# tky823/audio_source_separation

Hardware: AMD Instinct MI355X
Metric: ILRMA iterations/sec (4ch, F=1025, T=4096) (higher is better)
Workload: dtype f64; 1 GPU; gauss_ilrma_ip update_once, M=4 F=1025 T=4096 K=4, normalize=power, loss off; utterances_per_gpu=1, power_statistic=covariance, parallelism=utterance-sharded x1, no data-path collective

## Files before the change

### audio_source_separation_amd/csrc/assx_bss.hip

```cpp
#include "assx_common.hpp"
#include "assx_small_linalg.hpp"
#include "assx_stream.hpp"
#include "assx_group_linalg.hpp"
#include "assx_partition.hpp"
#include "assx_cov_wide.hpp"
#include "assx_cov_mfma.hpp"
#include "assx_nmf_internal.hpp"
#include "assx_widem.hpp"

using namespace assx;

namespace {

constexpr int REDUCE_THREADS = 256;

template <typename R, int M>
__device__ __forceinline__ void load_filter(const Cx<R>* __restrict__ W, size_t bf, Cx<R> (&w)[M][M]) {
  const Cx<R>* p = W + bf * (M * M);
#pragma unroll
  for (int n = 0; n < M; ++n)
#pragma unroll
    for (int m = 0; m < M; ++m) w[n][m] = p[n * M + m];
}

// ... 701 lines not shown
    for (int n = 0; n < N; ++n)
      Xi[((size_t)b * N + n) * FT + (size_t)(f0 + j) * T + t] =
          fma(nu, floor_eps<R>(r[n][j], eps), (R)2 * cabs2(y[n])) * inv;
  }
}

template <typename R>
__global__ void __launch_bounds__(256) pow_map_kernel(const R* __restrict__ in, R* __restrict__ out, size_t n, PowSpec p) {
  const size_t i = (size_t)blockIdx.x * blockDim.x + threadIdx.x;
  if (i < n) out[i] = powspec<R>(in[i], p);
}
template <typename R>
__global__ void __launch_bounds__(256) mix_variance_kernel(const R* __restrict__ Lambda, const R* __restrict__ g,
                                                          R* __restrict__ out, int M, int N, int F, int T) {
  const int t = blockIdx.x * blockDim.x + threadIdx.x, f = blockIdx.y, b = blockIdx.z;
  if (t >= T) return;
  const size_t FT = (size_t)F * T;
  for (int m = 0; m < M; ++m) {
    R acc = 0;
    for (int n = 0; n < N; ++n)
      acc += Lambda[((size_t)b * N + n) * FT + (size_t)f * T + t] * g[(((size_t)b * N + n) * F + f) * M + m];
    out[((size_t)b * M + m) * FT + (size_t)f * T + t] = acc;
  }
}

struct WsLayout {
  size_t part;
  size_t u;
  size_t lpart;
  size_t small;
  size_t map;
  size_t nmf;
  size_t tmp;
  size_t total;
};

constexpr int CHIP_CUS = 256;

inline long long g_target(int wgs_per_cu) {
  static const int rounds = lab_int("ASSX_ROUNDS", 1);
  const int forced = knob_int("ASSX_G", 0);
  if (forced > 0) return forced;
  return (long long)CHIP_CUS * wgs_per_cu * (rounds < 1 ? 1 : rounds);
}

inline int tblocks(int T) { return (T + WAVE - 1) / WAVE; }

template <typename R, int M>
constexpr int cov_lane_split() { return 1; }
inline FlatPart flat_cov(int B, int F, int T, int LS) {
  const int fb = WAVE / LS, tbk = (T + fb - 1) / fb;
  return make_flat(B, (long long)F * tbk, tbk, g_target(8));
}
inline FlatPart flat_basis(int B, int F, int T) {
  return make_flat(B, (long long)F * tblocks(T), tblocks(T), g_target(8));
}
inline FlatPart flat_act(int B, int F, int T) {
  return make_flat(B, (long long)tblocks(T) * F, F, g_target(8 / ACT_NH));
}

inline FlatPart flat_cov_wide(int B, int F, int T, int sb = 1) {
  const int tbk = (T + WAVE * sb - 1) / (WAVE * sb);
  return make_flat(B, (long long)((F + COVW_BINS - 1) / COVW_BINS) * tbk, tbk, g_target(1));
}
template <typename R>
inline int cov_wide_sb(int NK) {
// ... 22 lines not shown
  size_t pmax = p_cov;
  if (K > KU) {
    for (int sb = 1; sb <= 2; ++sb) {
      const FlatPart fw = flat_cov_wide(B, F, T, sb);
      const size_t p_wide = (size_t)fw.G * fw.S * COVW_BINS * (M * M * M);
      if (p_wide > pmax) pmax = p_wide;
    }
    const size_t p_adapt = (size_t)B * tblocks(T) * M * 2 * Kc * WAVE;
    if (p_adapt > pmax) pmax = p_adapt;
  }
  if (p_basis > pmax) pmax = p_basis;
  if (p_act > pmax) pmax = p_act;
  if (p_pb > pmax) pmax = p_pb;
  if (p_pow > pmax) pmax = p_pow;
  if (p_aux > pmax) pmax = p_aux;
  WsLayout L;
  L.part = 0;
  size_t off = align_up(pmax * r, 256);
  L.u = off;
  off += align_up((size_t)B * M * F * M * M * 2 * r, 256);
  L.lpart = off;
  size_t nl = (size_t)B * ((size_t)TS * F + (size_t)M * F + (size_t)M * ((T + 63) / 64) + F + 16 +
                           (size_t)flat_loss(F, T).G);
  off += align_up(nl * 8, 256);
  L.small = off;
  off += align_up((size_t)B * (M + 8) * 8, 256);
  L.map = L.nmf = L.tmp = off;
  if (K > KU) {
    off += align_up((size_t)B * M * F * T * r, 256);
    L.nmf = off;
    off += align_up(assx_nmf_workspace_bytes(B * M, F, T, K, dtype), 256);
    L.tmp = off;
    off += align_up(((size_t)B * M * F * K + (size_t)B * M * K * T) * r, 256);
  }
  L.total = off;
  return L;
}

template <typename Fn>
int dispatch_rm(assx_ctx* ctx, int dtype, int M, Fn&& fn) {
  if (dtype == ASSX_F64) {
    switch (M) {
#if !defined(ASSX_DEV_ONLY_M4_F64) && !defined(ASSX_DEV_ONLY_M4_F32)
      case 2: return fn(double(), IntC<2>());
      case 3: return fn(double(), IntC<3>());
#endif
#if !defined(ASSX_DEV_ONLY_M4_F32)
      case 4: return fn(double(), IntC<4>());
#endif
    }
  } else if (dtype == ASSX_F32) {
#if !defined(ASSX_DEV_ONLY_M4_F64)
    switch (M) {
#if !defined(ASSX_DEV_ONLY_M4_F32)
      case 2: return fn(float(), IntC<2>());
      case 3: return fn(float(), IntC<3>());
#endif
      case 4: return fn(float(), IntC<4>());
    }
#endif
  } else {
    return fail(ctx, ASSX_E_ARG, "dtype must be ASSX_F32 or ASSX_F64, got %d", dtype);
  }
  return fail(ctx, ASSX_E_UNSUPPORTED,
              "this entry point supports 2 <= M <= 4 channels, got M=%d (5 <= M <= 32 runs on the wide-channel path of the "
              "model entry points; more than 32 channels are not supported)", M);
// ... 116 lines not shown
int run_iss(assx_ctx* ctx, const void* U, const void* part, FlatPart fp, int T, void* W, const void* C, double* pw,
            int B, int F, hipStream_t st) {
  constexpr int GPW = WAVE / next_pow2_c(M * M);
  const dim3 grid(blocks_for((size_t)B * F, GPW)), block(64);
  if (part)
    hipLaunchKernelGGL((iss_group_kernel<R, M, true>), grid, block, 0, st, (const Cx<R>*)nullptr, (const R*)part, fp,
                       1.0 / (double)T, (double)T, (Cx<R>*)W, (const Cx<R>*)C, pw, B, F);
  else
    hipLaunchKernelGGL((iss_group_kernel<R, M, false>), grid, block, 0, st, (const Cx<R>*)U, (const R*)nullptr, fp, 1.0,
                       (double)T, (Cx<R>*)W, (const Cx<R>*)C, pw, B, F);
  ASSX_LAUNCH_CHECK(ctx, "iss_group_kernel");
  return 0;
}

template <typename R, int M>
int run_ip2(assx_ctx* ctx, const void* U, const void* part, FlatPart fp, int T, void* W, const void* C, double* pw,
            double thr, int32_t* status, int B, int F, int pm, int pn, hipStream_t st) {
  constexpr int GPW = WAVE / next_pow2_c(M * M);
  const dim3 grid(blocks_for((size_t)B * F, GPW)), block(64);
  if (part)
    hipLaunchKernelGGL((ip2_group_kernel<R, M, true>), grid, block, 0, st, (const Cx<R>*)nullptr, (const R*)part, fp,
                       1.0 / (double)T, (Cx<R>*)W, (const Cx<R>*)C, pw, thr, status, B, F, pm, pn);
  else
    hipLaunchKernelGGL((ip2_group_kernel<R, M, false>), grid, block, 0, st, (const Cx<R>*)U, (const R*)nullptr, fp, 1.0,
                       (Cx<R>*)W, (const Cx<R>*)C, pw, thr, status, B, F, pm, pn);
  ASSX_LAUNCH_CHECK(ctx, "ip2_group_kernel");
  return 0;
}

template <typename R, int MM>
int run_basis_partial(assx_ctx* ctx, const void* X, const void* W, const void* Tb, const void* V, double domain,
                      double eps, void* ws, int B, int F, int T, int K, hipStream_t st, FlatPart* fp_out,
                      double nu = -1.0 ,
                      double* lpart = nullptr , int lstride = 0) {
  NmfArgs<R> a;
  a.nu = (R)nu;
  a.d = Dims{B, F, T, K};
  a.eps = (R)eps;
  a.p1 = make_pow((domain + 2.0) / domain);
  a.fp = flat_basis(B, F, T);
  *fp_out = a.fp;
  const bool d2 = a.p1.mode == POW_SQUARE, k4 = K <= KU;
  const dim3 gb(stream_grid(ctx, a.fp, B)), bb(64);
#define BASIS_LAUNCH(K4V, D2V, DXV, DWV, MW) \
  hipLaunchKernelGGL((basis_stream_kernel<R, MM, K4V, D2V, DXV, DWV, MW>), gb, bb, 0, st, (const Cx<R>*)X, \
                     (const Cx<R>*)W, (const R*)Tb, (const R*)V, (R*)ws, a)
  constexpr size_t vlds = (size_t)VDMA_SLOTS * VTileDma<R, MM * KU>::TILE_BYTES;
#define BASIS_VD(D2V, MW, TDV) \
  hipLaunchKernelGGL((basis_stream_vd_kernel<R, MM, D2V, 2, MW, TDV>), gb, bb, vlds, st, (const Cx<R>*)X, \
                     (const Cx<R>*)W, (const R*)Tb, (const R*)V, (R*)ws, a, (double*)nullptr, 0)
#if ASSX_LAB
  static const int vdma = lab_int("ASSX_BASIS_VDMA", 1);
  if (k4 && !vdma) {
    if (nu >= 0.0) hipLaunchKernelGGL((basis_stream_kernel<R, MM, true, true, 3, 1, 1, true>), gb, bb, 0, st, (const Cx<R>*)X,
                                      (const Cx<R>*)W, (const R*)Tb, (const R*)V, (R*)ws, a);
    else if (d2) BASIS_LAUNCH(true, true, 3, 1, 2);
    else BASIS_LAUNCH(true, false, 2, 1, 1);
  } else
#endif
  if (nu >= 0.0) {
    if (k4) BASIS_VD(true, 2, true);
    else hipLaunchKernelGGL((basis_stream_kernel<R, MM, false, true, 3, 1, 1, true>), gb, bb, 0, st, (const Cx<R>*)X,
                            (const Cx<R>*)W, (const R*)Tb, (const R*)V, (R*)ws, a);
  } else if (k4) {
    if (d2 && lpart)
      hipLaunchKernelGGL((basis_stream_vd_kernel<R, MM, true, 2, 2, false, true>), gb, bb, vlds, st, (const Cx<R>*)X,
                         (const Cx<R>*)W, (const R*)Tb, (const R*)V, (R*)ws, a, lpart, lstride);
    else if (d2) BASIS_VD(true, 2, false);
    else BASIS_VD(false, 1, false);
  } else if (d2) BASIS_LAUNCH(false, true, 3, 1, 1);
  else BASIS_LAUNCH(false, false, 2, 1, 1);
#undef BASIS_VD
#undef BASIS_LAUNCH
  ASSX_LAUNCH_CHECK(ctx, "basis_stream_kernel");
  return 0;
}

template <typename R, int MM>
int run_act_partial(assx_ctx* ctx, const void* X, const void* W, const void* Tb, const void* V, double domain,
                    double eps, void* ws, int B, int F, int T, int K, hipStream_t st, FlatPart* fp_out,
                    double nu = -1.0) {
  NmfArgs<R> a;
  a.nu = (R)nu;
  a.d = Dims{B, F, T, K};
  a.eps = (R)eps;
  a.p1 = make_pow((domain + 2.0) / domain);
  a.fp = flat_act(B, F, T);
  *fp_out = a.fp;
  const bool d2 = a.p1.mode == POW_SQUARE, k4 = K <= KU;
  const dim3 ga(stream_grid(ctx, a.fp, B)), ba(64 * ACT_NH);
#define ACT_LAUNCH(K4V, D2V, DXV, MW) \
  hipLaunchKernelGGL((act_stream_kernel<R, MM, K4V, D2V, DXV, MW>), ga, ba, 0, st, (const Cx<R>*)X, (const Cx<R>*)W, \
                     (const R*)Tb, (const R*)V, (R*)ws, a)
#define ACT_VD(D2V, DXV, MW, TDV) \
  hipLaunchKernelGGL((act_stream_vd_kernel<R, MM, D2V, DXV, MW, TDV>), ga, ba, 0, st, (const Cx<R>*)X, (const Cx<R>*)W, \
                     (const R*)Tb, (const R*)V, (R*)ws, a)
#if ASSX_LAB
  static const int vdma = lab_int("ASSX_ACT_VDMA", 1);
  if (k4 && !vdma) {
    if (nu >= 0.0) hipLaunchKernelGGL((act_stream_kernel<R, MM, true, true, 3, 1, true>), ga, ba, 0, st, (const Cx<R>*)X,
                                      (const Cx<R>*)W, (const R*)Tb, (const R*)V, (R*)ws, a);
    else if (d2) ACT_LAUNCH(true, true, (sizeof(R) == 8 ? 3 : 4), 2);
    else ACT_LAUNCH(true, false, 2, 1);
  } else
#endif
  if (nu >= 0.0) {
    if (k4) ACT_VD(true, 3, 2, true);
    else hipLaunchKernelGGL((act_stream_kernel<R, MM, false, true, 4, 1, true>), ga, ba, 0, st, (const Cx<R>*)X,
                            (const Cx<R>*)W, (const R*)Tb, (const R*)V, (R*)ws, a);
  } else if (k4) {
    if (d2) ACT_VD(true, 3, 2, false);
    else ACT_VD(false, 2, 1, false);
  } else if (d2) ACT_LAUNCH(false, true, 4, 1);
  else ACT_LAUNCH(false, false, 2, 1);
#undef ACT_VD
#undef ACT_LAUNCH
  ASSX_LAUNCH_CHECK(ctx, "act_stream_kernel");
  return 0;
}

template <typename R, int MM>
int run_cov_partial_tv(assx_ctx* ctx, const void* X, const void* Tb, const void* V, int K, double domain, double eps,
                       void* ws, void* U_dense, int B, int F, int T, int dtype, hipStream_t st, FlatPart* fp_out,
                       bool* dense, int* records_wb = nullptr ) {
  static const bool wide = lab_int("ASSX_WIDE_K", 1) != 0;
  static const bool fused = lab_int("ASSX_COV_WIDE", 1) != 0;
  *dense = false;
  if (records_wb) *records_wb = 1;
  if (K <= KU || !wide) return run_cov_partial<R, MM>(ctx, WK_TV, X, nullptr, Tb, V, K, domain, eps, ws, B, F, T, st, fp_out);
  const WsLayout L = ws_layout(B, MM, F, T, K, dtype);
  const PowSpec p2d = make_pow(2.0 / domain);
  static const bool mfma = lab_int("ASSX_COV_MFMA", 1) != 0;
  if (fused && mfma && U_dense && K <= 16 && (size_t)B * MM * K * T * sizeof(R) < 0xffffffffull) {
    const FlatPart fw = flat_cov_wide(B, F, T, 1);
    const Dims d{B, F, T, K};
    const int ks = (K + 3) / 4;
    const size_t ldsm = CovMfmaGeom<R>::lds_bytes(MM, ks);
    unsigned long long* covm_trace = COVM_TRACE ? (unsigned long long*)((char*)ws + L.total - 65536) : nullptr;
#define COVM_LAUNCH(D2V, KSV)                                                                                          \
  do {                                                                                                                 \
    if (ldsm > 64 * 1024) {                                                                                            \
      hipError_t e = hipFuncSetAttribute(reinterpret_cast<const void*>(cov_mfma_kernel<R, MM, D2V, KSV>),              \
                                         hipFuncAttributeMaxDynamicSharedMemorySize, (int)ldsm);                       \
      if (e != hipSuccess) return hip_fail(ctx, e, "hipFuncSetAttribute(cov_mfma_kernel)");                            \
// ... 252 lines not shown
      if (!have_map) {
        rc = nmf_update_xfed(ctx, ASSX_NMF_IS_MM, domain, 0.0, eps, X, W, Tb, V, (char*)ws + L.nmf, B, MM, F, T, K, dtype, st);
        if (rc != ASSX_E_UNSUPPORTED) return rc;
        hipLaunchKernelGGL((demix_power_map_kernel<R, MM>), dim3(blocks_for(T, 256), F, B), dim3(256), 0, st,
                           (const Cx<R>*)X, (const Cx<R>*)W, pw, Dims{B, F, T, 0});
        ASSX_LAUNCH_CHECK(ctx, "demix_power_map_kernel");
      }
      NmfGroupScope grp(ctx, MM);
      return assx_nmf_update(ctx, ASSX_NMF_IS_MM, domain, eps, pw, Tb, V, (char*)ws + L.nmf, B * MM, F, T, K, dtype,
                             stream);
    }
    if (K > KU && wide_k && !full_mask && (source_mask & ((1u << MM) - 1u)) != 0u) {
      const WsLayout L = ws_layout(B, MM, F, T, K, dtype);
      R* pw = (R*)((char*)ws + L.map);
      const size_t nT = (size_t)B * MM * F * K, nV = (size_t)B * MM * K * T;
      R* Tt = (R*)((char*)ws + L.tmp);
      R* Vt = Tt + nT;
      if (!have_map) {
        hipLaunchKernelGGL((demix_power_map_kernel<R, MM>), dim3(blocks_for(T, 256), F, B), dim3(256), 0, st,
                           (const Cx<R>*)X, (const Cx<R>*)W, pw, Dims{B, F, T, 0});
        ASSX_LAUNCH_CHECK(ctx, "demix_power_map_kernel");
      }
      hipError_t e = hipMemcpyAsync(Tt, Tb, nT * sizeof(R), hipMemcpyDeviceToDevice, st);
      if (e == hipSuccess) e = hipMemcpyAsync(Vt, V, nV * sizeof(R), hipMemcpyDeviceToDevice, st);
      if (e != hipSuccess) return fail(ctx, (int)e, "hipMemcpyAsync(model copy): %s", hipGetErrorString(e));
      {
        NmfGroupScope grp(ctx, MM);
        rc = assx_nmf_update(ctx, ASSX_NMF_IS_MM, domain, eps, pw, Tt, Vt, (char*)ws + L.nmf, B * MM, F, T, K, dtype, stream);
      }
      if (rc) return rc;
      hipLaunchKernelGGL((masked_model_copy_kernel<R>), dim3(blocks_for(nT + nV, 256)), dim3(256), 0, st, (const R*)Tt,
                         (const R*)Vt, (R*)Tb, (R*)V, B, MM, (size_t)F * K, (size_t)K * T, source_mask);
      ASSX_LAUNCH_CHECK(ctx, "masked_model_copy_kernel");
      return 0;
    }
    rc = run_basis_partial<R, MM>(ctx, X, W, Tb, V, domain, eps, ws, B, F, T, K, st, &fp, -1.0, lpart, lstride);
    if (rc) return rc;
    const unsigned nb_basis = blocks_for((size_t)B * MM * F * K, 256);
    if (lpart)
      hipLaunchKernelGGL((basis_stream_finalize_kernel<R, MM>), dim3(nb_basis + blocks_for((size_t)B * F, 256)), dim3(256), 0,
                         st, (const R*)ws, (R*)Tb, B, MM, F, K, fp, (R)eps, p2, source_mask, (int)nb_basis, (const Cx<R>*)W,
                         lpart, lstride, lstride - F, T);
    else
      hipLaunchKernelGGL((basis_stream_finalize_kernel<R>), dim3(nb_basis), dim3(256), 0, st, (const R*)ws, (R*)Tb, B, MM,
                         F, K, fp, (R)eps, p2, source_mask);
    ASSX_LAUNCH_CHECK(ctx, "basis_stream_finalize_kernel");
    FlatPart fpa;
    rc = run_act_partial<R, MM>(ctx, X, W, Tb, V, domain, eps, ws, B, F, T, K, st, &fpa);
    if (rc) return rc;
    const unsigned nb_act = (unsigned)((size_t)B * MM * K * tblocks(T));
    hipLaunchKernelGGL((act_stream_finalize_kernel<R>), dim3(nb_act + (lpart ? (unsigned)B : 0u)), dim3(256), 0, st,
                       (const R*)ws, (R*)V, B, MM, F, K, T, fpa, (R)eps, p2, source_mask, (int)nb_act, (const double*)lpart,
                       loss_prev, lstride - F, lstride);
    ASSX_LAUNCH_CHECK(ctx, "act_stream_finalize_kernel");
    return 0;
  });
}

int assx_ilrma_expand_partitioned(assx_ctx* ctx, const void* Z, const void* Tb, const void* V, void* Teff, void* Veff,
                                  int B, int M, int F, int T, int K, int dtype, void* stream) {
  CHECK_COMMON(ctx, B, M, F, T);
  ASSX_REQUIRE(ctx, Z && Tb && V && (Teff || Veff), ASSX_E_NULL, "assx_ilrma_expand_partitioned: NULL array");
  ASSX_REQUIRE(ctx, K >= 1, ASSX_E_ARG, "n_basis must be >= 1, got %d", K);
  hipStream_t st = (hipStream_t)stream;
  const size_t total = (size_t)B * M * F * K + (size_t)B * M * K * T;
  if (dtype == ASSX_F64)
// ... 678 lines not shown
```

### audio_source_separation_amd/csrc/assx_stream.hpp

```cpp
#pragma once
#include <cstdlib>
#include "assx_common.hpp"

namespace assx {

enum { WK_NONE = 0, WK_NT = 1, WK_NFT = 2, WK_TV = 3 };

constexpr int KU = 4;

struct Dims {
  int B, F, T, K;
};

struct FlatPart {
  long long NB;
  int len;
  int L;
  int G;
  int S;
  int Gu;
  int Ju;
  int P;
  int Gp;
  int rev;
// ... 29 lines not shown
__host__ __device__ __forceinline__ bool flat_local(const FlatPart& fp, unsigned gl, unsigned& lo, unsigned& n) {
  const unsigned L = (unsigned)fp.L;
  if (fp.P > 0) {
    const unsigned grp = gl / (unsigned)fp.P, part = gl - grp * (unsigned)fp.P, len = (unsigned)fp.len;
    const unsigned off = part * L;
    if (off >= len) return false;
    lo = grp * len + off;
    n = off + L < len ? L : len - off;
    return true;
  }
  const unsigned nb = (unsigned)fp.NB;
  lo = gl * L;
  if (lo >= nb) return false;
  n = lo + L < nb ? L : nb - lo;
  return true;
}

__host__ __device__ __forceinline__ void flat_range(const FlatPart& fp, int g, long long& q0, long long& q1) {
  const int b = g / fp.Gu;
  unsigned lo = 0, n = 0;
  if (!flat_local(fp, (unsigned)(g - b * fp.Gu), lo, n)) n = 0;
  q0 = (long long)b * fp.NB + lo;
  q1 = q0 + n;
}
__device__ __forceinline__ bool flat_start(const FlatPart& fp, int g, int& b, int& grp, int& item, int& n) {
  b = g / fp.Gu;
  unsigned lo, cnt;
  if (!flat_local(fp, (unsigned)(g - b * fp.Gu), lo, cnt)) return false;
  n = (int)cnt;
  grp = (int)(lo / (unsigned)fp.len);
  item = (int)(lo - (unsigned)grp * (unsigned)fp.len);
  return true;
}
__host__ __device__ __forceinline__ void flat_cover(const FlatPart& fp, long long j, int& g_lo, int& g_hi) {
  const int b = (int)(j / fp.Ju);
  const unsigned jl = (unsigned)(j - (long long)b * fp.Ju);
  if (fp.P > 0) {
    g_lo = b * fp.Gu + (int)(jl * (unsigned)fp.P);
    g_hi = g_lo + (fp.len + fp.L - 1) / fp.L - 1;
    return;
  }
  const unsigned lo = jl * (unsigned)fp.len;
  g_lo = b * fp.Gu + (int)(lo / (unsigned)fp.L);
  g_hi = b * fp.Gu + (int)((lo + (unsigned)fp.len - 1u) / (unsigned)fp.L);
}
__host__ __device__ __forceinline__ int flat_slot(const FlatPart& fp, long long j, int g) {
  if (fp.P > 0) return 0;
  const int b = g / fp.Gu, gl = g - b * fp.Gu;
  return (int)(j - (long long)b * fp.Ju) - (int)(((unsigned)gl * (unsigned)fp.L) / (unsigned)fp.len);
}

struct Cursor {
  int b, f, tb;
};
__device__ __forceinline__ void advance(Cursor& c, int TBk, int F) {
  if (++c.tb == TBk) {
    c.tb = 0;
    if (++c.f == F) {
      c.f = 0;
      ++c.b;
    }
  }
}

constexpr int N_XCD = 8;
__host__ __device__ __forceinline__ int xcd_local_range(int bid, int G) {
  const int x = bid % N_XCD, j = bid / N_XCD;
  const int q = G / N_XCD, r = G % N_XCD;
  return x * q + (x < r ? x : r) + j;
}

__host__ __device__ __forceinline__ int workgroup_range(int bid, int grid, const FlatPart& fp) {
  if (fp.Gp == 0) return xcd_local_range(bid, grid);
  const int Gp = fp.Gp, B = grid / Gp;
  int b = bid / Gp;
  const int r = bid - b * Gp;
  const int x = r % N_XCD, j = r / N_XCD;
  const int q = fp.Gu / N_XCD, rem = fp.Gu % N_XCD;
  const int cnt = q + (x < rem ? 1 : 0);
  if (j >= cnt) return -1;
  const int first = x * q + (x < rem ? x : rem);
  if (fp.rev) {
// ... 608 lines not shown
            }
            tv = floor_eps<R>(tv, a.eps);
            if (TD) P = t_harmonic<R>(P, tv, a.nu);
            R inv = fast_rcp(tv);
            R D = D2 ? P * inv * inv : P / powspec<R>(tv, a.p1);
            if (ragged && t >= T) {
              inv = 0;
              D = 0;
            }
#pragma unroll
            for (int kk = 0; kk < KU; ++kk) {
              acc[(n * KU + kk) * 2 + 0] = fma(D, v[n][kk], acc[(n * KU + kk) * 2 + 0]);
              acc[(n * KU + kk) * 2 + 1] = fma(inv, v[n][kk], acc[(n * KU + kk) * 2 + 1]);
            }
          }

          if (cc.tb == 0 || !more) {
            const R tot = wave_reduce_scatter<R, NV>(acc);
            const int i = scatter_index<NV>();
            const int slot = cur.b * F + cur.f - bf_first;
            const int n = i / (2 * KU), k = k0 + (i >> 1) % KU;
            if (scatter_leader<NV>() && i < NACC && k < K)
              part[(((size_t)g * a.fp.S + slot) * N + n) * (size_t)(2 * K) + k * 2 + (i & 1)] = tot;
#pragma unroll
            for (int q = 0; q < NV; ++q) acc[q] = 0;
            if (more) load_rows(cc);
          }
        }
      }
    }
  }
}

template <typename R, int M, bool D2, int DXT, int MINW, bool TD, bool LOSS = false>
__global__ void __launch_bounds__(64, MINW)
    basis_stream_vd_kernel(const Cx<R>* __restrict__ X, const Cx<R>* __restrict__ W, const R* __restrict__ Tb,
                           const R* __restrict__ V, R* __restrict__ part, NmfArgs<R> a, double* __restrict__ lpart,
                           int lstride) {
  static_assert(!LOSS || (D2 && !TD), "the fused loss is the domain-2 Gaussian one");
  constexpr int N = M;
  constexpr int NACC = N * KU * 2;
  constexpr int NV = next_pow2_c(NACC);
  static_assert(NV <= WAVE && DXT >= 2, "accumulators / ring depth");
  using VT = VTileDma<R, N * KU>;
  extern __shared__ __attribute__((aligned(16))) unsigned char vlds[];
  const int lane = threadIdx.x & (WAVE - 1);
  const int F = a.d.F, T = a.d.T, K = a.d.K, TBk = a.fp.len;
  const size_t FT = (size_t)F * T;
  const int g = workgroup_range((int)blockIdx.x, (int)gridDim.x, a.fp);
  if (g < 0) return;
  Cursor cc;
  int nblk;
  if (!flat_start(a.fp, g, cc.b, cc.f, cc.tb, nblk)) return;
  const int bf_first = cc.b * F + cc.f;
  Cursor px = cc, pw = cc;
  const unsigned x_row = (unsigned)FT * (unsigned)sizeof(Cx<R>);
  const unsigned t_row = (unsigned)T * (unsigned)sizeof(R);

  R acc[NV];
#pragma unroll
  for (int i = 0; i < NV; ++i) acc[i] = 0;
  double lacc = 0.0, lm = 1.0;
  int le = 0;

  auto issue_x_tied = [&](const Cursor& c, Vec2<R>(&x)[M]) {
    const int t = c.tb * WAVE + lane;
    const unsigned tc = (unsigned)(t < T ? t : T - 1);
    const buf_u4 rx = make_rsrc_words(X + (size_t)c.b * M * FT, ~(size_t)0);
    const unsigned voff = ((unsigned)c.f * (unsigned)T + tc) * (unsigned)sizeof(Cx<R>);
    unsigned so = 0;
    const unsigned step = sgpr_opaque(x_row);
#pragma unroll
// ... 134 lines not shown
        lterm += (double)(P * inv);
        lprod *= (double)tv;
      }
      inv *= live;
      D *= live;
#pragma unroll
      for (int kk = 0; kk < KU; ++kk) {
        acc[(n * KU + kk) * 2 + 0] = fma(D, v[kk], acc[(n * KU + kk) * 2 + 0]);
        acc[(n * KU + kk) * 2 + 1] = fma(inv, v[kk], acc[(n * KU + kk) * 2 + 1]);
      }
    }
    if (LOSS) {
      if (t < T) {
        lacc += lterm;
        int e;
        lm = frexp(lm * lprod, &e);
        le += e;
      }
      asm volatile("" : "+v"(lacc), "+v"(lm));
    }
    value_fence(acc);
    if (STEADY || it + DXT < nblk) {
      issue_x_tied(px, xq[j]);
      advance(px, TBk, F);
    }

    if (cc.tb == 0 || !more) {
      const R tot = wave_reduce_scatter<R, NV>(acc);
      const int i = scatter_index<NV>();
      const int slot = cur.b * F + cur.f - bf_first;
      const int n = i / (2 * KU), k = (i >> 1) % KU;
      if (scatter_leader<NV>() && i < NACC && k < K)
        part[(((size_t)g * a.fp.S + slot) * N + n) * (size_t)(2 * K) + k * 2 + (i & 1)] = tot;
#pragma unroll
      for (int q = 0; q < NV; ++q) acc[q] = 0;
      if (LOSS && (cc.b != cur.b || !more)) {
        double tot = lacc + (double)le * 0.6931471805599453 + log(lm);
        tot = wave_allreduce_sum<double>(tot);
        if (lane == 0) lpart[(size_t)cur.b * lstride + (g - cur.b * a.fp.Gu)] = tot;
        lacc = 0.0;
        lm = 1.0;
        le = 0;
      }
      if (more) load_rows(cc);
    }
  };

  int it0 = 0;
  if (2 * DXT <= nblk) {
    static_for<DXT>([&](auto jc) { block(jc, IntC<2>(), decltype(jc)::value); });
    it0 = DXT;
  }
  for (; it0 + 2 * DXT <= nblk; it0 += DXT)
    static_for<DXT>([&](auto jc) { block(jc, IntC<1>(), it0 + decltype(jc)::value); });
  for (; it0 < nblk; it0 += DXT)
    static_for<DXT>([&](auto jc) {
      if (it0 + decltype(jc)::value < nblk) block(jc, IntC<0>(), it0 + decltype(jc)::value);
    });
}

template <int M, typename R>
__device__ __forceinline__ double neg2T_logabsdet(const Cx<R>* __restrict__ W, size_t bf, int T);

__device__ __forceinline__ void strided_sum_256(const double* __restrict__ p, int n, double& s) {
  for (int i0 = threadIdx.x; i0 < n; i0 += 256 * 8) {
    double v[8];
// ... 337 lines not shown
        le += e;
        if (TD) {
          tm = frexp(tm * tprod, &e);
          te += e;
        }
      }
      asm volatile("" : "+v"(acc), "+v"(lm), "+v"(tm));
      if (STEADY || it + DXT < nblk) {
        issue_x_tied(px, xq[j]);
        advance(px, TBk, F);
      }
      if (cc.tb == 0 && (STEADY || it + 1 < nblk)) load_rows(cc);
    };
    int it0 = 0;
    if (2 * DXT <= nblk) {
      static_for<DXT>([&](auto jc) { block(jc, IntC<2>(), decltype(jc)::value); });
      it0 = DXT;
    }
    for (; it0 + 2 * DXT <= nblk; it0 += DXT)
      static_for<DXT>([&](auto jc) { block(jc, IntC<1>(), it0 + decltype(jc)::value); });
    for (; it0 < nblk; it0 += DXT)
      static_for<DXT>([&](auto jc) {
        if (it0 + decltype(jc)::value < nblk) block(jc, IntC<0>(), it0 + decltype(jc)::value);
      });
  }
  acc += (double)le * 0.6931471805599453 + log(lm);
  if (TD) acc += (1.0 + 0.5 * (double)a.nu) * ((double)te * 0.6931471805599453 + log(tm));
  acc = wave_allreduce_sum<double>(acc);
  if (lane == 0) lpart[(size_t)b * lstride + g] = acc;
}

constexpr int ACT_NH = 4;

template <typename R, int M, bool K4, bool D2, int DXT, int MINW = 1, bool TD = false>
__global__ void __launch_bounds__(64 * ACT_NH, MINW)
    act_stream_kernel(const Cx<R>* __restrict__ X, const Cx<R>* __restrict__ W, const R* __restrict__ Tb,
                      const R* __restrict__ V, R* __restrict__ part, NmfArgs<R> a) {
  constexpr int N = M;
  constexpr int NACC = N * KU * 2;
  __shared__ R lds[(ACT_NH - 1) * NACC * WAVE];
  const int lane = threadIdx.x & (WAVE - 1);
  const int h = __builtin_amdgcn_readfirstlane(threadIdx.x >> 6);
  const int F = a.d.F, T = a.d.T, K = a.d.K;
  const int TBk = (T + WAVE - 1) / WAVE;
  const size_t FT = (size_t)F * T;
  const int g = workgroup_range((int)blockIdx.x, (int)gridDim.x, a.fp);
  if (g < 0) return;
  long long q0, q1;
  flat_range(a.fp, g, q0, q1);
  if (q0 >= q1) return;
  const long long bt_first = q0 / F;
  const long long bt_last = (q1 - 1) / F;
  const int nchunks = K4 ? 1 : (K + KU - 1) / KU;

  for (int c = 0; c < nchunks; ++c) {
    const int k0 = c * KU;
    for (long long bt = bt_first; bt <= bt_last; ++bt) {
      const int b = (int)(bt / TBk), tb = (int)(bt - (long long)b * TBk);
      const int fa = (int)((q0 > bt * F ? q0 : bt * F) - bt * F);
      const int fb = (int)((q1 < (bt + 1) * F ? q1 : (bt + 1) * F) - bt * F);
      const int t = tb * WAVE + lane;
      const bool valid = t < T;
      const unsigned tc = (unsigned)(valid ? t : T - 1);
      const Cx<R>* xb = X + (size_t)b * M * FT;
      const R* vb = V + (size_t)b * N * K * T;
      R v[N][KU];
// ... 36 lines not shown
            for (int n = 0; n < N; ++n) {
              Cx<R> y = cmake<R>(0, 0);
#pragma unroll
              for (int m = 0; m < M; ++m) cfma(y, wp[n * M + m], x[m]);
              R P = cabs2(y);
              const R* tbn = Tb + (((size_t)b * N + n) * F + f) * K;
              R tk[KU];
              R tv = 0;
              if (K4) {
#pragma unroll
                for (int kk = 0; kk < KU; ++kk) {
                  tk[kk] = (kk < K) ? tbn[kk] : (R)0;
                  tv = fma(tk[kk], v[n][kk], tv);
                }
              } else {
                const R* vn = vb + (size_t)n * K * T + tc;
                for (int k = 0; k < K; ++k) tv = fma(tbn[k], vn[(size_t)k * T], tv);
#pragma unroll
                for (int kk = 0; kk < KU; ++kk) tk[kk] = (k0 + kk < K) ? tbn[k0 + kk] : (R)0;
              }
              tv = floor_eps<R>(tv, a.eps);
              if (TD) P = t_harmonic<R>(P, tv, a.nu);
              const R inv = fast_rcp(tv);
              const R D = D2 ? P * inv * inv : P / powspec<R>(tv, a.p1);
#pragma unroll
              for (int kk = 0; kk < KU; ++kk) {
                acc[(n * KU + kk) * 2 + 0] = fma(tk[kk], D, acc[(n * KU + kk) * 2 + 0]);
                acc[(n * KU + kk) * 2 + 1] = fma(tk[kk], inv, acc[(n * KU + kk) * 2 + 1]);
              }
            }
          }
        }
      }
      if (h > 0) {
#pragma unroll
        for (int i = 0; i < NACC; ++i) lds[((h - 1) * NACC + i) * WAVE + lane] = acc[i];
      }
      __syncthreads();
      if (h == 0) {
        const int slot = (int)(bt - bt_first);
        R* out = part + ((size_t)g * a.fp.S + slot) * (size_t)(N * 2 * K) * WAVE + lane;
#pragma unroll
        for (int i = 0; i < NACC; ++i) {
          R tot = acc[i];
#pragma unroll
          for (int hh = 1; hh < ACT_NH; ++hh) tot += lds[((hh - 1) * NACC + i) * WAVE + lane];
          const int n = i / (2 * KU), k = k0 + (i >> 1) % KU;
          if (k < K) out[(size_t)(n * 2 * K + k * 2 + (i & 1)) * WAVE] = tot;
        }
      }
      __syncthreads();
    }
  }
}

constexpr int ACT_RING_SLOT = 512;

template <typename R, int M, bool D2, int DXT, int MINW, bool TD>
__global__ void __launch_bounds__(64 * ACT_NH, MINW)
    act_stream_vd_kernel(const Cx<R>* __restrict__ X, const Cx<R>* __restrict__ W, const R* __restrict__ Tb,
                         const R* __restrict__ V, R* __restrict__ part, NmfArgs<R> a) {
  constexpr int N = M;
  constexpr int NACC = N * KU * 2;
  constexpr int NISS = 2 + M;
  static_assert(N * M * 2 * (int)sizeof(R) <= 256 && N * KU * (int)sizeof(R) <= 256, "ring slot layout");
  __shared__ R lds[(ACT_NH - 1) * NACC * WAVE];
  __shared__ __attribute__((aligned(16))) unsigned char ring[ACT_NH * DXT * ACT_RING_SLOT];
  const int lane = threadIdx.x & (WAVE - 1);
  const int h = __builtin_amdgcn_readfirstlane(threadIdx.x >> 6);
  const int F = a.d.F, T = a.d.T, K = a.d.K;
  const size_t FT = (size_t)F * T;
  const int g = workgroup_range((int)blockIdx.x, (int)gridDim.x, a.fp);
  if (g < 0) return;
  int b, tb_first, f_first, nitems;
  if (!flat_start(a.fp, g, b, tb_first, f_first, nitems)) return;
  const int tb_last = tb_first + (f_first + nitems - 1) / F;
  const int f_end = f_first + nitems - (tb_last - tb_first) * F;
  const unsigned x_row = (unsigned)FT * (unsigned)sizeof(Cx<R>);
  unsigned char* myring = ring + h * (DXT * ACT_RING_SLOT);
  const unsigned ring0 = (unsigned)(size_t)(__attribute__((address_space(3))) void*)myring;
  const int w_dwords = N * M * 2 * (int)sizeof(R) / 4;
  const unsigned voff_w = (unsigned)(lane < w_dwords ? lane : w_dwords - 1) * 4u;
  constexpr int DPV = (int)sizeof(R) / 4;
  const int tn = lane / (KU * DPV), tkk = (lane / DPV) % KU;
  const unsigned voff_t = (tn < N && tkk < K)
                              ? ((unsigned)tn * (unsigned)F * (unsigned)K + (unsigned)tkk) * (unsigned)sizeof(R) +
                                    (unsigned)(lane % DPV) * 4u
                              : 0xfffffff0u;

  for (int tb = tb_first; tb <= tb_last; ++tb) {
    const int fa = tb == tb_first ? f_first : 0;
    const int fb = tb == tb_last ? f_end : F;
    const int t = tb * WAVE + lane;
    const unsigned tc = (unsigned)(t < T ? t : T - 1);
    R v[N][KU];
    {
      const BufRsrc rv = make_rsrc(V + (size_t)b * N * K * T);
#pragma unroll
      for (int n = 0; n < N; ++n)
#pragma unroll
        for (int kk = 0; kk < KU; ++kk)
          v[n][kk] = buf_ld<R>(rv, tc * (unsigned)sizeof(R),
                               (unsigned)(n * K + (kk < K ? kk : K - 1)) * (unsigned)T * (unsigned)sizeof(R));
    }
    R acc[NACC];
#pragma unroll
    for (int i = 0; i < NACC; ++i) acc[i] = 0;

    const buf_u4 rx = make_rsrc_words(X + (size_t)b * M * FT, ~(size_t)0);
    const buf_u4 rw = make_rsrc_words(W + (size_t)b * F * N * M, ~(size_t)0);
    const buf_u4 rt = make_rsrc_words(Tb + (size_t)b * N * F * K, (size_t)N * F * K * sizeof(R));
    const int nmine = (fb - fa - h + ACT_NH - 1) / ACT_NH;
    auto issue_bin = [&](int f, int slot, Vec2<R>(&x)[M]) {
      const unsigned la = ring0 + (unsigned)slot * (unsigned)ACT_RING_SLOT;
      buf_dword_to_lds(la, rw, voff_w, (unsigned)f * (unsigned)(N * M * 2 * (int)sizeof(R)));
      buf_dword_to_lds(la + 256u, rt, voff_t, (unsigned)f * (unsigned)K * (unsigned)sizeof(R));
      const unsigned voff = ((unsigned)f * (unsigned)T + tc) * (unsigned)sizeof(Cx<R>);
      unsigned so = 0;
      const unsigned step = sgpr_opaque(x_row);
#pragma unroll
      for (int m = 0; m < M; ++m) {
        buf_ldv_tied(x[m], rx, voff, so);
        so += step;
      }
    };
    Vec2<R> xq[DXT][M];
#pragma unroll
    for (int j = 0; j < DXT; ++j)
      if (j < nmine) {
#pragma unroll
        for (int m = 0; m < M; ++m) xq[j][m] = Vec2<R>{0, 0};
        issue_bin(fa + h + j * ACT_NH, j, xq[j]);
      }
    asm volatile("s_waitcnt vmcnt(0)" ::: "memory");
#pragma unroll
    for (int n = 0; n < N; ++n) value_fence(v[n]);

    auto block = [&](auto jc, auto steady, const int it) {
      constexpr int j = decltype(jc)::value;
      constexpr bool STEADY = decltype(steady)::value;
      const int f = fa + h + it * ACT_NH;
      if (STEADY) wait_slot<(DXT - 1) * NISS>(xq[j]);
      else wait_slot<0>(xq[j]);
      Cx<R> x[M];
#pragma unroll
      for (int m = 0; m < M; ++m) x[m] = tocx<R>(xq[j][m]);
      const Cx<R>* lw = reinterpret_cast<const Cx<R>*>(myring + j * ACT_RING_SLOT);
      const R* lt = reinterpret_cast<const R*>(myring + j * ACT_RING_SLOT + 256);
#if ASSX_BATCH_RCP
      R tvn[N], invn[N];
#pragma unroll
      for (int n = 0; n < N; ++n) {
        R tv = 0;
#pragma unroll
        for (int kk = 0; kk < KU; ++kk) tv = fma(lt[n * KU + kk], v[n][kk], tv);
        tvn[n] = floor_eps<R>(tv, a.eps);
      }
      batch_rcp<N>(tvn, invn);
      asm volatile("" ::: "memory");
#endif
#pragma unroll
      for (int n = 0; n < N; ++n) {
        Cx<R> y = cmake<R>(0, 0);
#pragma unroll
        for (int m = 0; m < M; ++m) cfma(y, lw[n * M + m], x[m]);
        R P = cabs2(y);
        R tk[KU];
#if ASSX_BATCH_RCP
#pragma unroll
        for (int kk = 0; kk < KU; ++kk) tk[kk] = lt[n * KU + kk];
        const R tv = tvn[n];
        if (TD) P = t_harmonic<R>(P, tv, a.nu);
        const R inv = invn[n];
#else
        R tv = 0;
#pragma unroll
        for (int kk = 0; kk < KU; ++kk) {
          tk[kk] = lt[n * KU + kk];
          tv = fma(tk[kk], v[n][kk], tv);
        }
        tv = floor_eps<R>(tv, a.eps);
        if (TD) P = t_harmonic<R>(P, tv, a.nu);
        const R inv = fast_rcp(tv);
#endif
        const R D = D2 ? P * inv * inv : P / powspec<R>(tv, a.p1);
#pragma unroll
        for (int kk = 0; kk < KU; ++kk) {
          acc[(n * KU + kk) * 2 + 0] = fma(tk[kk], D, acc[(n * KU + kk) * 2 + 0]);
          acc[(n * KU + kk) * 2 + 1] = fma(tk[kk], inv, acc[(n * KU + kk) * 2 + 1]);
        }
        if (n + 1 < N && (n & 1)) __builtin_amdgcn_sched_barrier(0);
      }
      value_fence(acc);
      if (STEADY || it + DXT < nmine) issue_bin(f + DXT * ACT_NH, j, xq[j]);
    };
    int it0 = 0;
    for (; it0 + 2 * DXT <= nmine; it0 += DXT)
      static_for<DXT>([&](auto jc) { block(jc, BoolC<true>(), it0 + decltype(jc)::value); });
    for (; it0 < nmine; it0 += DXT)
      static_for<DXT>([&](auto jc) {
        if (it0 + decltype(jc)::value < nmine) block(jc, BoolC<false>(), it0 + decltype(jc)::value);
      });

    if (h > 0) {
#pragma unroll
      for (int i = 0; i < NACC; ++i) lds[((h - 1) * NACC + i) * WAVE + lane] = acc[i];
    }
    __syncthreads();
    if (h == 0) {
      const int slot = tb - tb_first;
      R* out = part + ((size_t)g * a.fp.S + slot) * (size_t)(N * 2 * K) * WAVE + lane;
#pragma unroll
      for (int i = 0; i < NACC; ++i) {
        R tot = acc[i];
#pragma unroll
        for (int hh = 1; hh < ACT_NH; ++hh) tot += lds[((hh - 1) * NACC + i) * WAVE + lane];
        const int n = i / (2 * KU), k = (i >> 1) % KU;
        if (k < K) out[(size_t)(n * 2 * K + k * 2 + (i & 1)) * WAVE] = tot;
      }
    }
    __syncthreads();
  }
}

template <typename R>
__global__ void __launch_bounds__(256) act_stream_finalize_kernel(const R* __restrict__ part, R* __restrict__ V, int B,
                                                                 int N, int F, int K, int T, FlatPart fp, R eps,
                                                                 PowSpec p2, unsigned src_mask, int nb_main = 0,
                                                                 const double* __restrict__ lpart = nullptr,
                                                                 double* __restrict__ loss = nullptr, int ncov = 0,
                                                                 int lstride = 0) {
  if (lpart != nullptr && (int)blockIdx.x >= nb_main) {
    __shared__ double sm[256];
    const int b = (int)blockIdx.x - nb_main;
    double s = 0.0;
    strided_sum_256(lpart + (size_t)b * lstride, ncov, s);
    strided_sum_256(lpart + (size_t)b * lstride + ncov, F, s);
    sm[threadIdx.x] = s;
    __syncthreads();
    for (int off = 128; off >= 1; off >>= 1) {
      if ((int)threadIdx.x < off) sm[threadIdx.x] += sm[threadIdx.x + off];
      __syncthreads();
    }
    if (threadIdx.x == 0) loss[b] = sm[0];
    return;
  }
  __shared__ R sn[4][WAVE], sd[4][WAVE];
  const int lane = threadIdx.x & (WAVE - 1), q = threadIdx.x >> 6;
  const int TBk = (T + WAVE - 1) / WAVE;
  const int tb = blockIdx.x % TBk;
  const int k = (blockIdx.x / TBk) % K;
  const int n = (blockIdx.x / (TBk * K)) % N;
  const int b = blockIdx.x / (TBk * K * N);
// ... 41 lines not shown
```

Measured before the change: 5658 iterations/s.

## Fold basis finalize into activation kernel and split cross-wave reduction

Adds an optional path where the basis kernel also records the previous T values, and the activation kernel rebuilds the new T rows from the basis partials into dynamic LDS. This skips the separate basis finalize launch and the per-bin T loads. The path is off unless a knob is set. Independently, the per-block combine of wave accumulators is spread so each of the four waves reduces and stores a quarter of the outputs instead of wave 0 doing all of it. The new combine runs by default, and the fold adds redundant per-block recomputation and LDS pressure.

```diff
diff --git a/audio_source_separation_amd/csrc/assx_bss.hip b/audio_source_separation_amd/csrc/assx_bss.hip
--- a/audio_source_separation_amd/csrc/assx_bss.hip
+++ b/audio_source_separation_amd/csrc/assx_bss.hip
@@ -757,6 +757,8 @@
   size_t map;
   size_t nmf;
   size_t tmp;
+  size_t brec;
+  size_t tprev;
   size_t total;
 };
 
@@ -845,6 +847,12 @@
     off += align_up(assx_nmf_workspace_bytes(B * M, F, T, K, dtype), 256);
     L.tmp = off;
     off += align_up(((size_t)B * M * F * K + (size_t)B * M * K * T) * r, 256);
+  }
+  L.brec = L.tprev = off;
+  if (K <= KU) {
+    off += align_up(p_basis * r, 256);
+    L.tprev = off;
+    off += align_up((size_t)B * M * F * Kc * r, 256);
   }
   L.total = off;
   return L;
@@ -1027,7 +1035,8 @@
 int run_basis_partial(assx_ctx* ctx, const void* X, const void* W, const void* Tb, const void* V, double domain,
                       double eps, void* ws, int B, int F, int T, int K, hipStream_t st, FlatPart* fp_out,
                       double nu = -1.0 ,
-                      double* lpart = nullptr , int lstride = 0) {
+                      double* lpart = nullptr , int lstride = 0,
+                      void* tprev = nullptr ) {
   NmfArgs<R> a;
   a.nu = (R)nu;
   a.d = Dims{B, F, T, K};
@@ -1061,6 +1070,9 @@
     if (d2 && lpart)
       hipLaunchKernelGGL((basis_stream_vd_kernel<R, MM, true, 2, 2, false, true>), gb, bb, vlds, st, (const Cx<R>*)X,
                          (const Cx<R>*)W, (const R*)Tb, (const R*)V, (R*)ws, a, lpart, lstride);
+    else if (d2 && tprev)
+      hipLaunchKernelGGL((basis_stream_vd_kernel<R, MM, true, 2, 2, false, false, true>), gb, bb, vlds, st, (const Cx<R>*)X,
+                         (const Cx<R>*)W, (const R*)Tb, (const R*)V, (R*)ws, a, (double*)nullptr, 0, (R*)tprev);
     else if (d2) BASIS_VD(true, 2, false);
     else BASIS_VD(false, 1, false);
   } else if (d2) BASIS_LAUNCH(false, true, 3, 1, 1);
@@ -1071,10 +1083,19 @@
   return 0;
 }
 
+constexpr int ACT_D2_DXT = 3;
+template <typename R, int MM>
+inline size_t act_fold_table_bytes(int B, int F, int T) {
+  const FlatPart fa = flat_act(B, F, T);
+  const int seg = fa.L < F ? fa.L : F;
+  const size_t tab = (size_t)seg * act_fold_bin_bytes<R, MM>();
+  return 2 * ((size_t)act_static_lds_bytes<R, MM>(ACT_D2_DXT) + tab) <= (size_t)160 * 1024 ? tab : 0;
+}
+
 template <typename R, int MM>
 int run_act_partial(assx_ctx* ctx, const void* X, const void* W, const void* Tb, const void* V, double domain,
                     double eps, void* ws, int B, int F, int T, int K, hipStream_t st, FlatPart* fp_out,
-                    double nu = -1.0) {
+                    double nu = -1.0, const ActFold<R>* fold = nullptr, size_t fold_lds = 0) {
   NmfArgs<R> a;
   a.nu = (R)nu;
   a.d = Dims{B, F, T, K};
@@ -1104,7 +1125,16 @@
     else hipLaunchKernelGGL((act_stream_kernel<R, MM, false, true, 4, 1, true>), ga, ba, 0, st, (const Cx<R>*)X,
                             (const Cx<R>*)W, (const R*)Tb, (const R*)V, (R*)ws, a);
   } else if (k4) {
-    if (d2) ACT_VD(true, 3, 2, false);
+    if (d2 && fold) {
+      auto kern = act_stream_vd_kernel<R, MM, true, ACT_D2_DXT, 2, false, true>;
+      if (act_static_lds_bytes<R, MM>(ACT_D2_DXT) + fold_lds > 64 * 1024) {
+        hipError_t e = hipFuncSetAttribute(reinterpret_cast<const void*>(kern), hipFuncAttributeMaxDynamicSharedMemorySize,
+                                           (int)fold_lds);
+        if (e != hipSuccess) return hip_fail(ctx, e, "hipFuncSetAttribute(act_stream_vd_kernel)");
+      }
+      hipLaunchKernelGGL(kern, ga, ba, fold_lds, st, (const Cx<R>*)X, (const Cx<R>*)W, (const R*)nullptr, (const R*)V,
+                         (R*)ws, a, *fold);
+    } else if (d2) ACT_VD(true, ACT_D2_DXT, 2, false);
     else ACT_VD(false, 2, 1, false);
   } else if (d2) ACT_LAUNCH(false, true, 4, 1);
   else ACT_LAUNCH(false, false, 2, 1);
@@ -1423,6 +1453,27 @@
       hipLaunchKernelGGL((masked_model_copy_kernel<R>), dim3(blocks_for(nT + nV, 256)), dim3(256), 0, st, (const R*)Tt,
                          (const R*)Vt, (R*)Tb, (R*)V, B, MM, (size_t)F * K, (size_t)K * T, source_mask);
       ASSX_LAUNCH_CHECK(ctx, "masked_model_copy_kernel");
+      return 0;
+    }
+    const size_t fold_lds = (K <= KU && domain == 2.0 && full_mask && !loss_prev && knob_int("ASSX_ACT_BASIS_FOLD", 0) != 0 &&
+                             lab_int("ASSX_BASIS_VDMA", 1) != 0 && lab_int("ASSX_ACT_VDMA", 1) != 0)
+                                ? act_fold_table_bytes<R, MM>(B, F, T)
+                                : 0;
+    if (fold_lds > 0) {
+      const WsLayout L = ws_layout(B, MM, F, T, K, dtype);
+      ActFold<R> fo;
+      fo.tprev = (const R*)((char*)ws + L.tprev);
+      fo.brec = (const R*)((char*)ws + L.brec);
+      fo.tb_out = (R*)Tb;
+      rc = run_basis_partial<R, MM>(ctx, X, W, Tb, V, domain, eps, (char*)ws + L.brec, B, F, T, K, st, &fo.fpb, -1.0, nullptr,
+                                    0, (char*)ws + L.tprev);
+      if (rc) return rc;
+      FlatPart fpa;
+      rc = run_act_partial<R, MM>(ctx, X, W, nullptr, V, domain, eps, ws, B, F, T, K, st, &fpa, -1.0, &fo, fold_lds);
+      if (rc) return rc;
+      hipLaunchKernelGGL((act_stream_finalize_kernel<R>), dim3((unsigned)((size_t)B * MM * K * tblocks(T))), dim3(256), 0, st,
+                         (const R*)ws, (R*)V, B, MM, F, K, T, fpa, (R)eps, p2, source_mask);
+      ASSX_LAUNCH_CHECK(ctx, "act_stream_finalize_kernel");
       return 0;
     }
     rc = run_basis_partial<R, MM>(ctx, X, W, Tb, V, domain, eps, ws, B, F, T, K, st, &fp, -1.0, lpart, lstride);
diff --git a/audio_source_separation_amd/csrc/assx_stream.hpp b/audio_source_separation_amd/csrc/assx_stream.hpp
--- a/audio_source_separation_amd/csrc/assx_stream.hpp
+++ b/audio_source_separation_amd/csrc/assx_stream.hpp
@@ -85,9 +85,7 @@
   item = (int)(lo - (unsigned)grp * (unsigned)fp.len);
   return true;
 }
-__host__ __device__ __forceinline__ void flat_cover(const FlatPart& fp, long long j, int& g_lo, int& g_hi) {
-  const int b = (int)(j / fp.Ju);
-  const unsigned jl = (unsigned)(j - (long long)b * fp.Ju);
+__host__ __device__ __forceinline__ void flat_cover_local(const FlatPart& fp, int b, unsigned jl, int& g_lo, int& g_hi) {
   if (fp.P > 0) {
     g_lo = b * fp.Gu + (int)(jl * (unsigned)fp.P);
     g_hi = g_lo + (fp.len + fp.L - 1) / fp.L - 1;
@@ -97,10 +95,18 @@
   g_lo = b * fp.Gu + (int)(lo / (unsigned)fp.L);
   g_hi = b * fp.Gu + (int)((lo + (unsigned)fp.len - 1u) / (unsigned)fp.L);
 }
+__host__ __device__ __forceinline__ void flat_cover(const FlatPart& fp, long long j, int& g_lo, int& g_hi) {
+  const int b = (int)(j / fp.Ju);
+  flat_cover_local(fp, b, (unsigned)(j - (long long)b * fp.Ju), g_lo, g_hi);
+}
+__host__ __device__ __forceinline__ int flat_slot_local(const FlatPart& fp, int jl, int gl) {
+  if (fp.P > 0) return 0;
+  return jl - (int)(((unsigned)gl * (unsigned)fp.L) / (unsigned)fp.len);
+}
 __host__ __device__ __forceinline__ int flat_slot(const FlatPart& fp, long long j, int g) {
   if (fp.P > 0) return 0;
   const int b = g / fp.Gu, gl = g - b * fp.Gu;
-  return (int)(j - (long long)b * fp.Ju) - (int)(((unsigned)gl * (unsigned)fp.L) / (unsigned)fp.len);
+  return flat_slot_local(fp, (int)(j - (long long)b * fp.Ju), gl);
 }
 
 struct Cursor {
@@ -775,12 +781,13 @@
   }
 }
 
-template <typename R, int M, bool D2, int DXT, int MINW, bool TD, bool LOSS = false>
+template <typename R, int M, bool D2, int DXT, int MINW, bool TD, bool LOSS = false, bool FOLD = false>
 __global__ void __launch_bounds__(64, MINW)
     basis_stream_vd_kernel(const Cx<R>* __restrict__ X, const Cx<R>* __restrict__ W, const R* __restrict__ Tb,
                            const R* __restrict__ V, R* __restrict__ part, NmfArgs<R> a, double* __restrict__ lpart,
-                           int lstride) {
+                           int lstride, R* __restrict__ tprev = nullptr) {
   static_assert(!LOSS || (D2 && !TD), "the fused loss is the domain-2 Gaussian one");
+  static_assert(!FOLD || M * KU <= WAVE, "one lane per (source, component) of the side table");
   constexpr int N = M;
   constexpr int NACC = N * KU * 2;
   constexpr int NV = next_pow2_c(NACC);
@@ -981,6 +988,14 @@
       const int n = i / (2 * KU), k = (i >> 1) % KU;
       if (scatter_leader<NV>() && i < NACC && k < K)
         part[(((size_t)g * a.fp.S + slot) * N + n) * (size_t)(2 * K) + k * 2 + (i & 1)] = tot;
+      if (FOLD) {
+        const int ql = (int)order_after((unsigned)lane, tot);
+        R told = 0;
+#pragma unroll
+        for (int q = 0; q < N * KU; ++q) told = (ql == q) ? tbr[q / KU][q % KU] : told;
+        const int tn = ql / KU, tk = ql % KU;
+        if (tn < N && tk < K) tprev[(((size_t)cur.b * N + tn) * F + cur.f) * K + tk] = told;
+      }
 #pragma unroll
       for (int q = 0; q < NV; ++q) acc[q] = 0;
       if (LOSS && (cc.b != cur.b || !more)) {
@@ -1384,6 +1399,38 @@
 
 constexpr int ACT_NH = 4;
 
+template <typename R, int NACC>
+__device__ __forceinline__ void act_combine_store(const R (&acc)[NACC], R* __restrict__ lds, int h, int lane,
+                                                  R* __restrict__ out, int K, int k0) {
+  static_assert(NACC % ACT_NH == 0, "accumulators per wave");
+  constexpr int NOWN = NACC / ACT_NH;
+  auto at = [&](int o, int hs, int il) -> R& {
+    return lds[(((o * (ACT_NH - 1) + (hs > o ? hs - 1 : hs)) * NOWN + il) * WAVE) + lane];
+  };
+  static_for<ACT_NH>([&](auto oc) {
+    constexpr int o = decltype(oc)::value;
+    if (h != o) {
+#pragma unroll
+      for (int il = 0; il < NOWN; ++il) at(o, h, il) = acc[o * NOWN + il];
+    }
+  });
+  __syncthreads();
+  static_for<ACT_NH>([&](auto oc) {
+    constexpr int o = decltype(oc)::value;
+    if (h == o) {
+#pragma unroll
+      for (int il = 0; il < NOWN; ++il) {
+        const int i = o * NOWN + il;
+        R tot = o == 0 ? acc[i] : at(o, 0, il);
+#pragma unroll
+        for (int hh = 1; hh < ACT_NH; ++hh) tot += (hh == o) ? acc[i] : at(o, hh, il);
+        const int n = i / (2 * KU), k = k0 + (i >> 1) % KU;
+        if (k < K) out[(size_t)(n * 2 * K + k * 2 + (i & 1)) * WAVE] = tot;
+      }
+    }
+  });
+}
+
 template <typename R, int M, bool K4, bool D2, int DXT, int MINW = 1, bool TD = false>
 __global__ void __launch_bounds__(64 * ACT_NH, MINW)
     act_stream_kernel(const Cx<R>* __restrict__ X, const Cx<R>* __restrict__ W, const R* __restrict__ Tb,
@@ -1486,40 +1533,102 @@
           }
         }
       }
-      if (h > 0) {
-#pragma unroll
-        for (int i = 0; i < NACC; ++i) lds[((h - 1) * NACC + i) * WAVE + lane] = acc[i];
+      {
+        const int slot = (int)(bt - bt_first);
+        act_combine_store<R, NACC>(acc, lds, h, lane,
+                                   part + ((size_t)g * a.fp.S + slot) * (size_t)(N * 2 * K) * WAVE + lane, K, k0);
       }
       __syncthreads();
-      if (h == 0) {
-        const int slot = (int)(bt - bt_first);
-        R* out = part + ((size_t)g * a.fp.S + slot) * (size_t)(N * 2 * K) * WAVE + lane;
-#pragma unroll
-        for (int i = 0; i < NACC; ++i) {
-          R tot = acc[i];
-#pragma unroll
-          for (int hh = 1; hh < ACT_NH; ++hh) tot += lds[((hh - 1) * NACC + i) * WAVE + lane];
-          const int n = i / (2 * KU), k = k0 + (i >> 1) % KU;
-          if (k < K) out[(size_t)(n * 2 * K + k * 2 + (i & 1)) * WAVE] = tot;
-        }
-      }
-      __syncthreads();
     }
   }
 }
 
 constexpr int ACT_RING_SLOT = 512;
 
-template <typename R, int M, bool D2, int DXT, int MINW, bool TD>
+template <typename R>
+struct ActFold {
+  const R* tprev;
+  const R* brec;
+  R* tb_out;
+  FlatPart fpb;
+};
+template <typename R, int N>
+constexpr int act_fold_bin_bytes() { return N * KU * (int)sizeof(R); }
+template <typename R, int M>
+constexpr int act_static_lds_bytes(int dxt) {
+  return (ACT_NH - 1) * M * KU * 2 * WAVE * (int)sizeof(R) + ACT_NH * dxt * ACT_RING_SLOT;
+}
+
+template <typename R, int N>
+__device__ __forceinline__ void act_fold_rows(const ActFold<R>& fo, int b, int F, int K, int fa, int nb, R eps,
+                                              bool store, R* __restrict__ table) {
+  const FlatPart& fp = fo.fpb;
+  auto rows = [&](auto full) {
+    constexpr bool FULL = decltype(full)::value;
+    for (int o = (int)threadIdx.x; o < nb * N; o += WAVE * ACT_NH) {
+      const int fl = o / N, n = o - fl * N, f = fa + fl;
+      int g_lo, g_hi;
+      flat_cover_local(fp, b, (unsigned)f, g_lo, g_hi);
+      const int slot_lo = flat_slot_local(fp, f, g_lo - b * fp.Gu);
+      const size_t ti = (((size_t)b * N + n) * F + f) * K;
+      R told[KU], num[KU], den[KU];
+#pragma unroll
+      for (int kk = 0; kk < KU; ++kk) {
+        told[kk] = (FULL || kk < K) ? fo.tprev[ti + kk] : (R)0;
+        num[kk] = den[kk] = 0;
+      }
+      constexpr int RC = 4;
+      for (int g0 = g_lo; g0 <= g_hi; g0 += RC) {
+        R vn[RC][KU], vd[RC][KU];
+#pragma unroll
+        for (int c = 0; c < RC; ++c) {
+          const int g = min(g0 + c, g_hi);
+          const R* p = fo.brec + (((size_t)g * fp.S + (g == g_lo ? slot_lo : 0)) * N + n) * (size_t)(2 * K);
+#pragma unroll
+          for (int kk = 0; kk < KU; ++kk) {
+            vn[c][kk] = (FULL || kk < K) ? p[kk * 2] : (R)0;
+            vd[c][kk] = (FULL || kk < K) ? p[kk * 2 + 1] : (R)0;
+          }
+        }
+#pragma unroll
+        for (int c = 0; c < RC; ++c)
+          if (g0 + c <= g_hi) {
+#pragma unroll
+            for (int kk = 0; kk < KU; ++kk) {
+              num[kk] += vn[c][kk];
+              den[kk] += vd[c][kk];
+            }
+          }
+      }
+#pragma unroll
+      for (int kk = 0; kk < KU; ++kk) {
+        R tnew = 0;
+        if (FULL || kk < K) {
+          tnew = told[kk] * sqrt(num[kk] / floor_eps<R>(den[kk], eps));
+          if (store) fo.tb_out[ti + kk] = tnew;
+        }
+        table[(fl * N + n) * KU + kk] = tnew;
+      }
+    }
+  };
+  if (K == KU) rows(BoolC<true>());
+  else rows(BoolC<false>());
+}
+
+template <typename R, int M, bool D2, int DXT, int MINW, bool TD, bool FOLD = false>
 __global__ void __launch_bounds__(64 * ACT_NH, MINW)
     act_stream_vd_kernel(const Cx<R>* __restrict__ X, const Cx<R>* __restrict__ W, const R* __restrict__ Tb,
-                         const R* __restrict__ V, R* __restrict__ part, NmfArgs<R> a) {
+                         const R* __restrict__ V, R* __restrict__ part, NmfArgs<R> a, ActFold<R> fo = ActFold<R>{}) {
   constexpr int N = M;
   constexpr int NACC = N * KU * 2;
-  constexpr int NISS = 2 + M;
+  constexpr int NISS = (FOLD ? 1 : 2) + M;
   static_assert(N * M * 2 * (int)sizeof(R) <= 256 && N * KU * (int)sizeof(R) <= 256, "ring slot layout");
+  static_assert(act_static_lds_bytes<R, M>(DXT) == (int)sizeof(R) * (ACT_NH - 1) * NACC * WAVE + ACT_NH * DXT * ACT_RING_SLOT,
+                "the host's figure for the static LDS");
   __shared__ R lds[(ACT_NH - 1) * NACC * WAVE];
   __shared__ __attribute__((aligned(16))) unsigned char ring[ACT_NH * DXT * ACT_RING_SLOT];
+  extern __shared__ __attribute__((aligned(16))) unsigned char fold_lds[];
+  R* const ttab = reinterpret_cast<R*>(fold_lds);
   const int lane = threadIdx.x & (WAVE - 1);
   const int h = __builtin_amdgcn_readfirstlane(threadIdx.x >> 6);
   const int F = a.d.F, T = a.d.T, K = a.d.K;
@@ -1568,7 +1677,7 @@
     auto issue_bin = [&](int f, int slot, Vec2<R>(&x)[M]) {
       const unsigned la = ring0 + (unsigned)slot * (unsigned)ACT_RING_SLOT;
       buf_dword_to_lds(la, rw, voff_w, (unsigned)f * (unsigned)(N * M * 2 * (int)sizeof(R)));
-      buf_dword_to_lds(la + 256u, rt, voff_t, (unsigned)f * (unsigned)K * (unsigned)sizeof(R));
+      if (!FOLD) buf_dword_to_lds(la + 256u, rt, voff_t, (unsigned)f * (unsigned)K * (unsigned)sizeof(R));
       const unsigned voff = ((unsigned)f * (unsigned)T + tc) * (unsigned)sizeof(Cx<R>);
       unsigned so = 0;
       const unsigned step = sgpr_opaque(x_row);
@@ -1586,9 +1695,11 @@
         for (int m = 0; m < M; ++m) xq[j][m] = Vec2<R>{0, 0};
         issue_bin(fa + h + j * ACT_NH, j, xq[j]);
       }
+    if (FOLD) act_fold_rows<R, N>(fo, b, F, K, fa, fb - fa, a.eps, tb == 0, ttab);
     asm volatile("s_waitcnt vmcnt(0)" ::: "memory");
 #pragma unroll
     for (int n = 0; n < N; ++n) value_fence(v[n]);
+    if (FOLD) __syncthreads();
 
     auto block = [&](auto jc, auto steady, const int it) {
       constexpr int j = decltype(jc)::value;
@@ -1600,7 +1711,7 @@
 #pragma unroll
       for (int m = 0; m < M; ++m) x[m] = tocx<R>(xq[j][m]);
       const Cx<R>* lw = reinterpret_cast<const Cx<R>*>(myring + j * ACT_RING_SLOT);
-      const R* lt = reinterpret_cast<const R*>(myring + j * ACT_RING_SLOT + 256);
+      const R* lt = FOLD ? ttab + (f - fa) * (N * KU) : reinterpret_cast<const R*>(myring + j * ACT_RING_SLOT + 256);
 #if ASSX_BATCH_RCP
       R tvn[N], invn[N];
 #pragma unroll
@@ -1656,23 +1767,8 @@
         if (it0 + decltype(jc)::value < nmine) block(jc, BoolC<false>(), it0 + decltype(jc)::value);
       });
 
-    if (h > 0) {
-#pragma unroll
-      for (int i = 0; i < NACC; ++i) lds[((h - 1) * NACC + i) * WAVE + lane] = acc[i];
-    }
-    __syncthreads();
-    if (h == 0) {
-      const int slot = tb - tb_first;
-      R* out = part + ((size_t)g * a.fp.S + slot) * (size_t)(N * 2 * K) * WAVE + lane;
-#pragma unroll
-      for (int i = 0; i < NACC; ++i) {
-        R tot = acc[i];
-#pragma unroll
-        for (int hh = 1; hh < ACT_NH; ++hh) tot += lds[((hh - 1) * NACC + i) * WAVE + lane];
-        const int n = i / (2 * KU), k = (i >> 1) % KU;
-        if (k < K) out[(size_t)(n * 2 * K + k * 2 + (i & 1)) * WAVE] = tot;
-      }
-    }
+    act_combine_store<R, NACC>(acc, lds, h, lane,
+                               part + ((size_t)g * a.fp.S + (tb - tb_first)) * (size_t)(N * 2 * K) * WAVE + lane, K, 0);
     __syncthreads();
   }
 }
```

After: 5663 iterations/s (median of 2 runs). No clear change (+0.1%).
